# cvlab-kaist/SOLA

Hardware: AMD Instinct MI355X
Metric: track-selection forward+loss samples/sec at (T=32,N=64,d=256) (higher is better)
Workload: dtype f32 via split-f16 (hi+lo f16 operand pairs, 3 f16 MFMAs per product, f32 accumulate); 1 GPU; SOLA track selection forward+BCE+alignment loss+selection, T=32 N=64 d=256 L=16, mevis/default model (32.98M params, random init), 256 samples/step/GPU, conv weights re-standardised every step; batch_per_gpu=256, tracks=64, frames=32, text_len=16

## Files before the change

### include/sola_hip.h

```cpp
#ifndef SOLA_HIP_H
#define SOLA_HIP_H

#include <stddef.h>
#include <stdint.h>

#ifdef __cplusplus
extern "C" {
#endif

typedef enum SolaStatus {
    SOLA_OK = 0,
    SOLA_ERR_ARG = -1,
    SOLA_ERR_HIP = -2,
    SOLA_ERR_WEIGHT = -3,
    SOLA_ERR_WORKSPACE = -4,
    SOLA_ERR_STATE = -5
} SolaStatus;

typedef struct SolaConfig {
    int32_t object_token_dim;
    int32_t lang_token_dim;
    int32_t n_layers;
    int32_t max_temporal_length;
    int32_t n_negative;
// ... 14 lines not shown
int sola_weight_info(const SolaCtx* ctx, int index, const char** name, int64_t* numel);

int sola_set_weight(SolaCtx* ctx, const char* name, const void* dev_ptr, int64_t numel);

int sola_weights_changed(SolaCtx* ctx);
int sola_set_ws_policy(SolaCtx* ctx, int recompute_every_forward);

int sola_set_precision(SolaCtx* ctx, int precision);
int sola_set_split_guard(SolaCtx* ctx, int enable);

int sola_set_x16_arena(SolaCtx* ctx, void* dev_ptr, size_t bytes);
int sola_x16_arena_info(const SolaCtx* ctx, size_t* need_bytes, size_t* capacity_bytes, size_t* used_bytes);
int sola_split_fallback_count(const SolaCtx* ctx, int64_t* count, int32_t* last_guard);
int sola_cast_sp16(const float* dev_in, int ld_in, float* dev_out, int ld_out, int64_t rows, int K, float scale, void* stream);
int sola_cast_sp16_auto(const float* dev_in, int ld_in, float* dev_out, int ld_out, int64_t rows, int K, float* dev_scal, void* stream);
int sola_gemm_nt_split(const float* dev_a_sp, int lda, const float* dev_w_sp, const float* dev_bias, const float* dev_r,
                       int ldr, int r_is_split, float* dev_c, int ldc, int c_is_split, int M, int N, int K, float out_scale,
                       void* stream);
int sola_gemm_nt_split_scaled(const float* dev_a_sp, int lda, const float* dev_w_sp, const float* dev_bias, const float* dev_r,
                              int ldr, int r_is_split, float* dev_c, int ldc, int c_is_split, int M, int N, int K,
                              float out_scale, const float* dev_out_scale, void* stream);

int sola_cast_f16(const float* dev_in, int ld_in, void* dev_out, int ld_out, int64_t rows, int K, float scale, float* dev_scal, void* stream);
int sola_gemm_nt_f16(const void* dev_a_h, int lda, const void* dev_w_h, const float* dev_bias, const void* dev_r_h, int ldr,
                     void* dev_c, int ldc, int c_is_f16, int M, int N, int K, float out_scale, void* stream);
int sola_attention_f16(const void* dev_q, int ldq, const void* dev_k, int ldk, const void* dev_v, int ldv, void* dev_o, int ldo,
                       int G, int H, int head_dim, int Sq, int Sk, int inner, int64_t q_outer, int64_t q_inner, int64_t q_row_stride,
                       int64_t k_outer, int64_t k_inner, int64_t k_row_stride, float scale, void* stream);

int sola_gemm_nt_bf16(const void* dev_a, int lda, const void* dev_w, const float* dev_bias, const void* dev_r, int ldr, int r_is_bf16,
// ... 35 lines not shown

int sola_workspace_tap(const SolaCtx* ctx, const char* name, size_t* byte_offset, int64_t* rows, int64_t* cols);

int sola_loss(const float* dev_score_map, const float* dev_score_tokens,
              const float* dev_labels,
              const float* dev_pos_tokens,
              const float* dev_neg_tokens, int64_t neg_batch_stride,
              int B, int N, int D, int n_neg,
              float positive_weight, float temperature, float alignment_weight,
              float* dev_loss3, int32_t* dev_neg_argmax,
              void* dev_scratch, size_t scratch_bytes, void* stream);

int sola_select(const float* dev_score_map, int64_t n, float threshold, float* dev_prob, float* dev_pred, void* stream);

int sola_ws_standardize(const float* dev_w, int cout, int cin, int k, float* dev_out, void* stream);
int sola_gemm_nt(const float* dev_a, int lda, const float* dev_w, const float* dev_bias, const float* dev_r, int ldr,
                 float* dev_c, int ldc, int M, int N, int K, void* stream);
int sola_gemm_nn(const float* dev_a, int lda, const float* dev_w0, const float* dev_w1, const float* dev_w2, int w_rows, const float* dev_r,
                 int ldr, float* dev_c, int ldc, int M, int N, int K, void* stream);
int sola_conv1d_cl(const float* dev_x, const float* dev_wstd, const float* dev_bias, float* dev_y,
                   int R, int T_in, int cin, int cout, int k, int stride, int pad, void* stream);
int sola_group_norm(const float* dev_x, float* dev_y, float* dev_y2, const float* dev_pe,
                    const float* dev_gamma, const float* dev_beta,
                    int n_inst, int inner, int64_t outer_stride, int64_t inner_stride, int64_t tok_stride,
                    int ntok, int C, int groups, float eps, float leaky_slope, int apply_leaky, void* stream);
int sola_attention(const float* dev_q, int ldq, const float* dev_k, int ldk, const float* dev_v, int ldv,
                   float* dev_o, int ldo, int G, int H, int head_dim, int Sq, int Sk, int inner,
                   int64_t q_outer, int64_t q_inner, int64_t q_row_stride,
                   int64_t k_outer, int64_t k_inner, int64_t k_row_stride, float scale,
                   float* dev_lse , void* stream);
// ... 197 lines not shown
```

### sola_amd/_lib.py

```python
from __future__ import annotations

import contextlib
import ctypes as C
import os

_HERE = os.path.dirname(os.path.abspath(__file__))
LIB_PATH = os.environ.get("SOLA_HIP_LIB") or os.path.join(_HERE, "lib", "libsola_hip.so")


class SolaLibraryError(RuntimeError):
    pass


class SolaError(RuntimeError):
    """A libsola_hip call returned a negative status."""


class SolaConfig(C.Structure):
    _fields_ = [
        ("object_token_dim", C.c_int32),
        ("lang_token_dim", C.c_int32),
        ("n_layers", C.c_int32),
        ("max_temporal_length", C.c_int32),
        ("n_negative", C.c_int32),
# ... 20 lines not shown
    "sola_last_error": (C.c_char_p, []),
    "sola_version": (C.c_char_p, []),
    "sola_ctx_create": (_i, [C.POINTER(SolaConfig), _i, C.POINTER(_vp)]),
    "sola_ctx_destroy": (_i, [_vp]),
    "sola_num_weights": (_i, [_vp]),
    "sola_weight_info": (_i, [_vp, _i, C.POINTER(C.c_char_p), C.POINTER(_i64)]),
    "sola_set_weight": (_i, [_vp, C.c_char_p, _vp, _i64]),
    "sola_weights_changed": (_i, [_vp]),
    "sola_set_ws_policy": (_i, [_vp, _i]),
    "sola_set_precision": (_i, [_vp, _i]),
    "sola_set_split_guard": (_i, [_vp, _i]),
    "sola_split_fallback_count": (_i, [_vp, C.POINTER(_i64), C.POINTER(C.c_int32)]),
    "sola_cast_sp16": (_i, [_vp, _i, _vp, _i, _i64, _i, _f, _vp]),
    "sola_gemm_nt_split": (_i, [_vp, _i, _vp, _vp, _vp, _i, _i, _vp, _i, _i, _i, _i, _i, _f, _vp]),
    "sola_cast_sp16_auto": (_i, [_vp, _i, _vp, _i, _i64, _i, _vp, _vp]),
    "sola_gemm_nt_split_scaled": (_i, [_vp, _i, _vp, _vp, _vp, _i, _i, _vp, _i, _i, _i, _i, _i, _f, _vp, _vp]),
    "sola_cast_f16": (_i, [_vp, _i, _vp, _i, _i64, _i, _f, _vp, _vp]),
    "sola_gemm_nt_f16": (_i, [_vp, _i, _vp, _vp, _vp, _i, _vp, _i, _i, _i, _i, _i, _f, _vp]),
    "sola_gemm_nn": (_i, [_vp, _i, _vp, _vp, _vp, _i, _vp, _i, _vp, _i, _i, _i, _i, _vp]),
    "sola_gemm_nt_bf16": (_i, [_vp, _i, _vp, _vp, _vp, _i, _i, _vp, _i, _i, _i, _i, _i, _vp]),
    "sola_attention_bf16": (_i, [_vp, _i, _vp, _i, _vp, _i, _vp, _vp, _i, _i, _i, _i, _i, _i, _i, _i64, _i64, _i64, _i64, _i64, _i64, _f, _vp, _vp]),
    "sola_attention_backward_bf16": (_i, [_vp, _i, _vp, _i, _vp, _i, _vp, _i, _vp, _i, _i, _vp, _vp, _vp, _vp, _i, _i, _i, _vp, _vp, _i, _i, _i, _i, _i, _i,
                                          _i64, _i64, _i64, _i64, _i64, _i64, _f, _i64, _vp, _sz, _vp]),
    "sola_attention_f16": (_i, [_vp, _i, _vp, _i, _vp, _i, _vp, _i, _i, _i, _i, _i, _i, _i, _i64, _i64, _i64, _i64, _i64, _i64, _f, _vp]),
    "sola_workspace_bytes": (_sz, [_vp, _i, _i, _i, _i]),
    "sola_forward": (_i, [_vp, _vp, _vp, _i, _i, _i, _i, _vp, _vp, _vp, _sz, _vp]),
    "sola_ragged_workspace_bytes": (_sz, [_vp, C.POINTER(SolaRaggedBatch)]),
    "sola_forward_ragged": (_i, [_vp, _vp, _vp, C.POINTER(SolaRaggedBatch), _vp, _vp, _vp, _sz, _vp]),
    "sola_loss_ragged": (_i, [_vp, _vp, _vp, _vp, _vp, _i64, _i, _vp, _i, _i64, _i, _i, _f, _f, _f, _vp, _vp, _vp, _sz, _vp]),
    "sola_train_ragged_workspace_bytes": (_sz, [_vp, C.POINTER(SolaRaggedBatch)]),
    "sola_backward_ragged_workspace_bytes": (_sz, [_vp, C.POINTER(SolaRaggedBatch)]),
    "sola_forward_train_ragged": (_i, [_vp, _vp, _vp, C.POINTER(SolaRaggedBatch), _vp, _vp, _vp, _sz, _vp]),
    "sola_backward_ragged": (_i, [_vp, _vp, _vp, _vp, _vp, _sz, _vp]),
    "sola_loss_backward_ragged": (_i, [_vp, _vp, _vp, _vp, _vp, _i64, _i, _vp, _i, _i64, _i, _i, _f, _f, _f, _vp, _vp, _vp, _vp, _vp, _sz, _vp]),
    "sola_workspace_tap": (_i, [_vp, C.c_char_p, C.POINTER(_sz), C.POINTER(_i64), C.POINTER(_i64)]),
    "sola_loss": (_i, [_vp, _vp, _vp, _vp, _vp, _i64, _i, _i, _i, _i, _f, _f, _f, _vp, _vp, _vp, _sz, _vp]),
    "sola_select": (_i, [_vp, _i64, _f, _vp, _vp, _vp]),
    "sola_ws_standardize": (_i, [_vp, _i, _i, _i, _vp, _vp]),
    "sola_gemm_nt": (_i, [_vp, _i, _vp, _vp, _vp, _i, _vp, _i, _i, _i, _i, _vp]),
    "sola_conv1d_cl": (_i, [_vp, _vp, _vp, _vp, _i, _i, _i, _i, _i, _i, _i, _vp]),
    "sola_group_norm": (_i, [_vp, _vp, _vp, _vp, _vp, _vp, _i, _i, _i64, _i64, _i64, _i, _i, _i, _f, _f, _i, _vp]),
    "sola_attention": (_i, [_vp, _i, _vp, _i, _vp, _i, _vp, _i, _i, _i, _i, _i, _i, _i, _i64, _i64, _i64, _i64, _i64, _i64, _f, _vp, _vp]),
    "sola_attention_split": (_i, [_vp, _i, _vp, _i, _vp, _i, _vp, _i, _i, _i, _i, _i, _i, _i, _i, _i64, _i64, _i64, _i64, _i64, _i64, _f, _vp, _vp]),
    "sola_set_dropout": (_i, [_vp, _f, _f, C.c_uint64]),
    "sola_set_stage_dropout": (_i, [_f, C.c_uint64]),
    "sola_train_workspace_bytes": (_sz, [_vp, _i, _i, _i, _i]),
    "sola_backward_workspace_bytes": (_sz, [_vp, _i, _i, _i, _i]),
    "sola_set_grad": (_i, [_vp, C.c_char_p, _vp, _i64]),
    "sola_forward_train": (_i, [_vp, _vp, _vp, _i, _i, _i, _i, _vp, _vp, _vp, _sz, _vp]),
    "sola_backward": (_i, [_vp, _vp, _vp, _vp, _vp, _sz, _vp]),
    "sola_grad_bucket_count": (_i, [_vp]),
    "sola_grad_bucket_of": (_i, [_vp, C.c_char_p]),
    "sola_backward_wait_bucket": (_i, [_vp, _i, _vp]),
# ... 171 lines not shown
```

### sola_amd/csrc/api.hip

```cpp
#include <math.h>
#include <stdarg.h>
#include <string.h>

#include <algorithm>
#include <exception>
#include <mutex>

#include "ragged.h"
#include "tune.h"

static thread_local char g_err[1024] = "";
void sola_set_error(const char* fmt, ...) {
    va_list ap;
    va_start(ap, fmt);
    vsnprintf(g_err, sizeof(g_err), fmt, ap);
    va_end(ap);
}
extern "C" const char* sola_last_error(void) { return g_err; }
extern "C" const char* sola_version(void) { return "sola_hip 0.6 (gfx950; f32, range-guarded split-f16 and f16-operand MFMA forward and backward, ragged batches, mask IoU + masklet rows)"; }

namespace {
struct ProfRec {
    int cat;
    hipEvent_t e0, e1;
// ... 357 lines not shown
    if (rows) *rows = it->second.rows;
    if (cols) *cols = it->second.cols;
    return SOLA_OK;
}

extern "C" int sola_set_precision(SolaCtx* c, int precision) {
    SOLA_ARG(c && precision >= 0 && precision <= 3, "set_precision: 0 (f32), 1 (split-f16), 2 (f16 storage / f16 GEMM operands) or 3 (bf16 GEMM operands, training)");
    if (precision >= 1 && !c->lin16_buf) {
        const size_t D = c->cfg.lang_token_dim;
        size_t ws_total = 0;
        for (int i = 0; i < 6; ++i) ws_total += (size_t)c->conv[i].cout * c->conv[i].cin * c->conv[i].k;
        SOLA_HIP(hipSetDevice(c->device));
        SOLA_HIP(hipMalloc(&c->ws16_buf, ws_total * sizeof(float)));
        SOLA_HIP(hipMalloc(&c->lin16_buf, (size_t)c->cfg.n_layers * 12 * D * D * sizeof(float)));
        const size_t n_pairs = 2 + (size_t)c->cfg.n_layers * 12;
        SOLA_HIP(hipMalloc(&c->scal_buf, (2 * n_pairs + 2 + 4) * sizeof(float)));
        SOLA_HIP(hipMemset(c->scal_buf, 0, (2 * n_pairs + 2 + 4) * sizeof(float)));
        c->guard = reinterpret_cast<int*>(c->scal_buf + 2 * n_pairs);
        SOLA_HIP(hipHostMalloc(reinterpret_cast<void**>(&c->guard_host), 2 * sizeof(int), hipHostMallocDefault));
        c->guard_host[0] = c->guard_host[1] = 0;
    }
    c->precision = precision;
    c->ws_dirty = true;
    c->lin16_dirty = true;
    return SOLA_OK;
}

extern "C" int sola_cast_sp16(const float* in, int ld_in, float* out, int ld_out, int64_t rows, int K, float scale, void* stream_) {
    return launch_cast_sp16(in, ld_in, out, ld_out, rows, K, scale, as_stream(stream_));
}

extern "C" int sola_gemm_nt_split(const float* a_sp, int lda, const float* w_sp, const float* bias, const float* r, int ldr,
// ... 59 lines not shown
                                            int64_t q_rs, int64_t k_outer, int64_t k_inner, int64_t k_rs, float scale, int64_t q_rows, float* scratch,
                                            size_t scratch_floats, void* stream_) {
    SOLA_ARG(q && k && v && o && dout && lse && dq16 && dk16 && dv16 && dq_scratch && dvec, "attention_backward_bf16: null argument");
    AttnBwdDesc d{static_cast<const float*>(q), static_cast<const float*>(k), static_cast<const float*>(v), static_cast<const float*>(o), static_cast<const float*>(dout), lse, dq_scratch, nullptr, nullptr, dvec,
                  ldq, ldk, ldv, ldo, ld_dq, ld_dk, ld_dv, G, H, head_dim, Sq, Sk, inner, q_outer, q_inner, q_rs, k_outer, k_inner, k_rs, scale};
    d.drop = g_stage_drop;
    d.part = scratch; d.part_floats = scratch_floats; d.part_rows = q_rows;
    d.io_bf16 = 1; d.dq16 = dq16; d.dk16 = dk16; d.dv16 = dv16;
    d.dout_bf16 = dout_bf16 ? 1 : 0;
    d.o_bf16 = o_bf16 ? 1 : 0;
    return launch_attention_bwd(d, as_stream(stream_));
}

extern "C" int sola_cast_sp16_auto(const float* in, int ld_in, float* out, int ld_out, int64_t rows, int K, float* scal, void* stream_) {
    return launch_cast_sp16_auto(in, ld_in, out, ld_out, rows, K, scal, as_stream(stream_));
}

extern "C" int sola_gemm_nt_split_scaled(const float* a_sp, int lda, const float* w_sp, const float* bias, const float* r, int ldr,
                                         int r_sp16, float* cmat, int ldc, int c_sp16, int M, int N, int K, float out_scale,
                                         const float* out_scale_dev, void* stream_) {
    SOLA_ARG(a_sp && w_sp && cmat, "gemm_nt_split_scaled: null argument");
    GemmDesc gd{};
    gd.nprob = 1;
    gd.p[0] = GemmProblem{a_sp, w_sp, bias, r, cmat};
    gd.M = M; gd.N = N; gd.K = K; gd.lda = lda; gd.ldr = ldr; gd.ldc = ldc;
    gd.arith = 1; gd.out_scale = out_scale; gd.out_scale_dev = out_scale_dev; gd.r_sp16 = r_sp16; gd.c_sp16 = c_sp16;
    return launch_gemm(gd, as_stream(stream_));
}

int sola_split_guard_tripped(SolaCtx* c, hipStream_t s, bool* tripped) {
// ... 256 lines not shown

extern "C" int sola_grad_clip(float* const* dev_grads, const int64_t* numel, int n, const double* dev_total_sq,
                              float max_norm, void* stream_) {
    SOLA_ARG(dev_grads && numel && dev_total_sq, "grad_clip: null argument");
    return launch_mt_clip(dev_grads, reinterpret_cast<const long long*>(numel), n, dev_total_sq, max_norm, as_stream(stream_));
}

extern "C" int sola_select(const float* score, int64_t n, float thr, float* prob, float* pred, void* stream_) {
    SOLA_ARG(score && (prob || pred), "select: null argument");
    return launch_select(score, n, thr, prob, pred, as_stream(stream_));
}

extern "C" int sola_ws_standardize(const float* w, int cout, int cin, int k, float* out, void* stream_) {
    SOLA_ARG(w && out && cout > 0, "ws_standardize: bad argument");
    WsLayer l{w, out, cout, cin, k};
    return launch_ws_standardize(&l, 1, as_stream(stream_));
}

extern "C" int sola_ws_backward(const float* w, const float* dwstd, int cout, int cin, int k, float* dw, void* stream_) {
    SOLA_ARG(w && dwstd && dw && cout > 0, "ws_backward: bad argument");
    WsBwdLayer l{w, dwstd, dw, cout, cin, k};
    return launch_ws_backward(&l, 1, as_stream(stream_));
}

extern "C" int sola_gemm_nt(const float* a, int lda, const float* w, const float* bias, const float* r, int ldr,
                            float* cmat, int ldc, int M, int N, int K, void* stream_) {
    SOLA_ARG(a && w && cmat, "gemm_nt: null argument");
    GemmDesc gd{};
    gd.nprob = 1;
    gd.p[0] = GemmProblem{a, w, bias, r, cmat};
// ... 424 lines not shown
```

### sola_amd/csrc/cast.hip

```cpp
#include <algorithm>

#include "kernels.h"

namespace {

typedef _Float16 half8 __attribute__((ext_vector_type(8)));

__global__ __launch_bounds__(256) void cast_sp16_kernel(const float* __restrict__ in, float* __restrict__ out, long long rows,
                                                        int blocks_per_row, int ld_in, int ld_out, float scale, _Float16* __restrict__ side) {
    const long long i = (long long)blockIdx.x * blockDim.x + threadIdx.x;
    if (i >= rows * blocks_per_row) return;
    const long long r = i / blocks_per_row;
    const int b = (int)(i - r * blocks_per_row);
    const float4 v0 = *reinterpret_cast<const float4*>(in + r * ld_in + b * 8);
    const float4 v1 = *reinterpret_cast<const float4*>(in + r * ld_in + b * 8 + 4);
    const float v[8] = {v0.x * scale, v0.y * scale, v0.z * scale, v0.w * scale, v1.x * scale, v1.y * scale, v1.z * scale, v1.w * scale};
    half8 hi, lo;
#pragma unroll
    for (int j = 0; j < 8; ++j) {
        _Float16 h1, l1;
        split_f16(v[j], h1, l1);
        hi[j] = h1; lo[j] = l1;
    }
    half8* o = reinterpret_cast<half8*>(out + r * ld_out + b * 8);
// ... 120 lines not shown
    const long long r = i / blocks_per_row;
    const int b = (int)(i - r * blocks_per_row);
    const float4 v0 = *reinterpret_cast<const float4*>(in + r * ld_in + b * 8);
    const float4 v1 = *reinterpret_cast<const float4*>(in + r * ld_in + b * 8 + 4);
    const float v[8] = {v0.x * scale, v0.y * scale, v0.z * scale, v0.w * scale, v1.x * scale, v1.y * scale, v1.z * scale, v1.w * scale};
    half8 hi, lo;
#pragma unroll
    for (int j = 0; j < 8; ++j) {
        _Float16 h1, l1;
        split_f16(v[j], h1, l1);
        hi[j] = h1; lo[j] = l1;
    }
    half8* o = reinterpret_cast<half8*>(out + r * ld_out + b * 8);
    o[0] = hi;
    o[1] = lo;
}

constexpr int MULTI_MAX = 64;
struct MultiArgs {
    const float* in[MULTI_MAX];
    float* out[MULTI_MAX];
};
__global__ __launch_bounds__(256) void amax_multi_kernel(const MultiArgs a, unsigned* __restrict__ scal, long long n4) {
    const float* in = a.in[blockIdx.z];
    float m = 0.f;
    for (long long i = (long long)blockIdx.x * 256 + threadIdx.x; i < n4; i += (long long)gridDim.x * 256) {
        const float4 v = *reinterpret_cast<const float4*>(in + i * 4);
        m = fmaxf(m, fmaxf(fmaxf(fabsf(v.x), fabsf(v.y)), fmaxf(fabsf(v.z), fabsf(v.w))));
    }
    block_amax_commit(m, scal + 2 * blockIdx.z);
// ... 228 lines not shown
    SolaProfScope prof(SOLA_PROF_MISC, s, 0, 12.0 * rows * K);
    SOLA_HIP(hipMemsetAsync(scal, 0, 2 * sizeof(float), s));
    {
        long long ar = rows; int ak = K, ald = ld_in;
        amax_shape(ar, ak, ald);
        hipLaunchKernelGGL(amax_kernel, dim3((unsigned)((ak / 4 + 255) / 256), (unsigned)((ar + 63) / 64)), dim3(256), 0, s, in,
                           reinterpret_cast<unsigned*>(scal), ar, ak / 4, ald);
    }
    SOLA_LAUNCH_CHECK();
    const long long n = rows * (K / 8);
    hipLaunchKernelGGL(cast_sp16_auto_kernel, dim3((unsigned)((n + 255) / 256)), dim3(256), 0, s, in, out, rows, K / 8, ld_in, ld_out, scal);
    SOLA_LAUNCH_CHECK();
    return SOLA_OK;
}

int launch_cast_sp16(const float* in, int ld_in, float* out, int ld_out, long long rows, int K, float scale, hipStream_t s, void* side16) {
    SOLA_ARG(in && out && rows > 0 && K > 0 && K % 8 == 0 && ld_in % 4 == 0 && ld_out % 8 == 0, "cast_sp16: K=%d ld_in=%d ld_out=%d", K, ld_in, ld_out);
    const long long n = rows * (K / 8);
    SolaProfScope prof(SOLA_PROF_MISC, s, 0, (side16 ? 10.0 : 8.0) * rows * K);
    hipLaunchKernelGGL(cast_sp16_kernel, dim3((unsigned)((n + 255) / 256)), dim3(256), 0, s, in, out, rows, K / 8, ld_in, ld_out, scale,
                       static_cast<_Float16*>(side16));
    SOLA_LAUNCH_CHECK();
    return SOLA_OK;
}
```

### sola_amd/csrc/ctx.h

```cpp
#pragma once
#include <string>
#include <unordered_map>
#include <vector>

#include "kernels.h"

struct ConvGeom {
    int cin, cout, k, stride, pad;
};
struct Weight {
    std::string name;
    int64_t numel;
    const float* ptr;
    float* grad;
};
struct Buf {
    size_t off;
    int64_t rows, cols;
};
struct Plan {
    int B = 0, N = 0, T = 0, L = 0, W = 0, Tp = 0, M = 0;
    int Tl[6] = {0};
    bool train = false;
    bool rag = false;
// ... 70 lines not shown
    }
    float* scal_buf = nullptr;
    int* guard = nullptr;
    int* guard_host = nullptr;
    bool split_guard = true;
    long long split_fallbacks = 0;
    bool weight_range_bad = false;
    SolaRagStage* rag_stage = nullptr;
    std::vector<hipEvent_t> bucket_ev;
    hipStream_t side_stream = nullptr;
    hipEvent_t ev_fork = nullptr, ev_side[4] = {nullptr, nullptr, nullptr, nullptr};
    bool bucket_recorded = false;
    int n_buckets() const { return cfg.n_layers + 1; }
    float* scal_pair(int i) const { return scal_buf + 2 * i; }
    float* scal_extra(int i) const { return scal_buf + 2 * (2 + (size_t)cfg.n_layers * 12) + 2 + i; }
    const float* lin_inv_scale(int layer, int attn, int proj) const { return scal_buf + 2 * (2 + (layer * 3 + attn) * 4 + proj) + 1; }
    struct StepBinding {
        std::vector<int> widx;
        std::vector<int32_t> group;
        std::vector<long long> numel;
        int n_groups = 0;
        size_t sq_scratch = 0;
    } step;
    void* adam_tab = nullptr;
    int adam_n = 0, adam_cap = 0, adam_blocks = 0;
    bool adam_has_steps = false;
    int* adam_ticket = nullptr;
    double adam_bytes = 0.0;
    float p_drop_encoder = 0.f, p_drop_attention = 0.f;
    unsigned long long drop_seed = 0;
// ... 39 lines not shown
```

### sola_amd/csrc/forward_infer.hip

```cpp
#include <math.h>

#include <algorithm>

#include "ragged.h"

int sola_refresh_lin16(SolaCtx* c, hipStream_t s) {
    if (!c->lin16_dirty) return SOLA_OK;
    SOLA_ARG(c->lin16_buf && c->scal_buf, "split-f16 weights requested before sola_set_precision(ctx, 1)");
    static const char* pn[4] = {"q_proj", "k_proj", "v_proj", "out_proj"};
    const int D = c->cfg.lang_token_dim;
    std::vector<const float*> in;
    std::vector<float*> out;
    for (int l = 0; l < c->cfg.n_layers; ++l)
        for (int a = 0; a < 3; ++a)
            for (int j = 0; j < 4; ++j) {
                const std::string nm = "object_lang_align_layers." + std::to_string(l) + "." + kAttnLong[a] + "." + pn[j] + ".weight";
                const float* w = ctx_weight(c, nm);
                if (!w) {
                    sola_set_error("forward: weight '%s' has not been set", nm.c_str());
                    return SOLA_ERR_WEIGHT;
                }
                in.push_back(w);
                out.push_back(c->lin16_buf + ((size_t)(l * 3 + a) * 4 + j) * D * D);
            }
// ... 20 lines not shown
            return SOLA_ERR_WEIGHT;
        }
    SOLA_HIP(hipMemsetAsync(c->guard + 1, 0, sizeof(int), s));
    for (size_t i0 = 0; i0 < norms.size(); i0 += 32)
        SOLA_TRY(launch_norm_range_check(norms.data() + i0, (int)std::min<size_t>(32, norms.size() - i0), c->guard + 1, s));
    c->lin16_dirty = false;
    return SOLA_OK;
}

int sola_refresh_conv_weights(SolaCtx* c, int fmt, bool force, hipStream_t s) {
    if (!force && !c->ws_dirty && !c->ws_every_forward && (fmt == 0 || c->ws16_fmt == fmt)) return SOLA_OK;
    WsLayer layers[6];
    for (int i = 0; i < 6; ++i) {
        const std::string nm = "short_motion_encoder." + std::to_string(kConvIdx[i]) + ".weight";
        layers[i] = WsLayer{ctx_weight(c, nm), c->ws_buf + c->ws_off[i], c->conv[i].cout, c->conv[i].cin, c->conv[i].k};
    }
    SOLA_TRY(launch_ws_standardize(layers, 6, s));
    c->ws16_fmt = 0;
    for (int i = 0; i < 6 && fmt != 0; ++i) {
        const int kc = c->conv[i].k * c->conv[i].cin;
        const float* w = c->ws_buf + c->ws_off[i];
        if (fmt == 1) SOLA_TRY(launch_cast_sp16(w, kc, c->ws16_buf + c->ws_off[i], kc, c->conv[i].cout, kc, 1.f, s));
        else SOLA_TRY(launch_cast_f16(w, kc, reinterpret_cast<_Float16*>(c->ws16_buf) + c->ws_off[i], kc, c->conv[i].cout, kc, 1.f, nullptr, s, 13,
                                      nullptr, fmt == 3 ? 1 : 0));
    }
    c->ws_dirty = false;
    c->ws16_fmt = fmt;
    return SOLA_OK;
}

int sola_check_forward_args(const SolaCtx* c, const char* who, size_t need, const void* workspace, size_t ws_bytes) {
    for (const Weight& w : c->weights)
        if (!w.ptr) {
            sola_set_error("%s: weight '%s' has not been set", who, w.name.c_str());
            return SOLA_ERR_WEIGHT;
        }
// ... 63 lines not shown
    }
    std::string lin_name(int layer, int attn_i, int proj) const {
        return "object_lang_align_layers." + std::to_string(layer) + "." + kAttnLong[attn_i] + "." + kProj[proj];
    }
    GemmProblem lin_problem(const float* a, int layer, int attn_i, int proj, const float* r, float* out) const {
        const std::string nm = lin_name(layer, attn_i, proj);
        const size_t at = ((size_t)(layer * 3 + attn_i) * 4 + proj) * D * D;
        const float* w = sp ? c->lin16_buf + at
                       : h16 ? reinterpret_cast<const float*>(reinterpret_cast<const _Float16*>(c->lin16_buf) + at)
                             : W(nm + ".weight");
        return GemmProblem{a, w, W(nm + ".bias"), r, out, op16 ? c->lin_inv_scale(layer, attn_i, proj) : nullptr};
    }

    int cast_obj(const float* obj, float* obj_sp, long long rows) const {
        const int d_in = c->cfg.object_token_dim;
        if (sp) return launch_cast_sp16_auto(obj, d_in, obj_sp, d_in, rows, d_in, c->scal_pair(0), s);
        return launch_cast_f16(obj, d_in, obj_sp, d_in, rows, d_in, 256.f, c->scal_pair(0), s, 6, c->scal_extra(0));
    }
    int cast_lang(const float* lang, float* lang_sp, long long rows) const {
        if (sp) return launch_cast_sp16_auto(lang, D, lang_sp, D, rows, D, c->scal_pair(1), s);
        return launch_cast_f16(lang, D, lang_sp, D, rows, D, 1.f, c->scal_pair(1), s, 6);
    }
    const float* lang_inv_scale() const { return op16 ? c->scal_pair(1) + 1 : nullptr; }

    GemmDesc gemm(long long rows, int N, int K) const {
        GemmDesc gd{};
        gd.M = (int)rows; gd.N = N; gd.K = K; gd.ldc = N;
        if (op16) { gd.arith = sp ? 1 : 2; gd.out_scale = 1.f; }
        gd.splitk_ws = splitk_ws; gd.splitk_bytes = splitk_bytes;
        return gd;
    }
    GemmDesc conv_gemm(int i, const float* x, float* out, long long rows) const {
        const ConvGeom& g = c->conv[i];
        GemmDesc gd = gemm(rows, g.cout, g.k * g.cin);
        gd.nprob = 1;
// ... 376 lines not shown
```

### sola_amd/csrc/kernels.h

```cpp
#pragma once
#include "common.h"

struct GemmProblem {
    const float* A;
    const float* W;
    const float* bias;
    const float* R;
    float* C;
    const float* scale_dev;
};
struct GemmDesc {
    GemmProblem p[3];
    int nprob;
    int M, N, K;
    int lda, ldr, ldc;
    int conv;
    int T_in, T_out, stride, pad, Cin;
    const int2* rowmap;
    int arith;
    float out_scale;
    int ksplit;
    const float* out_scale_dev;
    int r_sp16;
    int c_sp16;
// ... 221 lines not shown

size_t mt_sqnorm_scratch_bytes(int n, const long long* numel);
int launch_mt_sqnorm(const float* const* ptrs, const long long* numel, const int* group, int n, int n_groups, double* out,
                     void* scratch, size_t scratch_bytes, hipStream_t s);
int launch_mt_clip(float* const* ptrs, const long long* numel, int n, const double* total_sq, float max_norm, hipStream_t s);
size_t mt_adam_entry_bytes();
void mt_adam_entry_fill(void* host_entry, float* p, float* g, float* m, float* v, float* step, long long numel, int first_block);
int mt_adam_blocks(long long numel);
int launch_mt_clip_adamw(const void* tab_dev, int n, int blocks, double bytes, const double* total_sq, float max_norm, double lr, double beta1, double beta2,
                         double eps, double weight_decay, float step, int write_back, int* ticket, hipStream_t s);

struct WsLayer {
    const float* w;
    float* out;
    int cout, cin, k;
};
int launch_ws_standardize(const WsLayer* layers, int n_layers, hipStream_t s);

struct GroupNormDesc {
    const float* x;
    float* y;
    float* y2;
    const float* pe;
    const float *gamma, *beta;
    int n_inst, inner;
    long long outer_stride, inner_stride, tok_stride;
    int ntok, C, groups;
    float eps, slope;
    int leaky;
    DropoutCfg drop;
// ... 6 lines not shown
    size_t slice_ws_bytes;
    void* y_cast = nullptr;
    void* y2_cast = nullptr;
    int cast_fmt = 0;
    void* stats_out = nullptr;
    int* stats_written = nullptr;
};
int launch_group_norm(const GroupNormDesc& d, hipStream_t s);
int launch_cast_sp16(const float* in, int ld_in, float* out, int ld_out, long long rows, int K, float scale, hipStream_t s, void* side16 = nullptr);
int launch_amax_accumulate(const float* in, int ld_in, long long rows, int K, float* scal, hipStream_t s);
int launch_amax_colsum(const float* in, int ld_in, long long rows, int K, float* scal, float* part, hipStream_t s);
int launch_cast_bf16_colsum(const float* in, int ld_in, void* out, int ld_out, long long rows, int K, float* scal, float* part, hipStream_t s);
int launch_colsum_slabs_bf16(const void* in, int ld_in, long long rows, int K, float* scal, float* part, hipStream_t s);
int launch_cast_sp16_scaled(const float* in, int ld_in, float* out, int ld_out, long long rows, int K, float* scal, hipStream_t s);
int launch_cast_sp16_auto(const float* in, int ld_in, float* out, int ld_out, long long rows, int K, float* scal, hipStream_t s);
int launch_cast_sp16_auto_multi(const float* const* in, float* const* out, int n, int rows, int K, float* scal, hipStream_t s);
int launch_cast_f16(const float* in, int ld_in, void* out, int ld_out, long long rows, int K, float scale, float* scal, hipStream_t s,
                    int target_exp = 13, float* scale_out = nullptr, int bf16 = 0);
int launch_cast_f16_auto_multi(const float* const* in, void* const* out, int n, int rows, int K, float* scal, hipStream_t s, int bf16 = 0);
int launch_cast_f16_scaled(const float* in, int ld_in, void* out, int ld_out, long long rows, int K, float* scal, hipStream_t s, int bf16 = 0);
int launch_cast_f16_t(const float* in, int ld_in, void* out, long long ld_out, int rows, int cols, float* scal, hipStream_t s, int bf16 = 0);
struct NormPair { const float *gamma, *beta; int C; };
int launch_norm_range_check(const NormPair* norms, int n, int* guard, hipStream_t s);
int launch_pos_encoding(const float* gauss, int D, int t_len, int max_len, float* pe, hipStream_t s);
int launch_lang_concat(const float* lang, const float* neg, float* out, float* lbar, int B, int L, int n_neg, int D,
                       hipStream_t s);
int launch_lang_concat_shared(const float* lang, const float* neg, float* out, float* lbar, int B, int L, int n_neg, int D, hipStream_t s);
int launch_lang_concat_ragged(const float* lang, const float* neg, float* out, float* lbar, int B, const int4* units, int n_neg,
                              int D, hipStream_t s);
int launch_gather_rows(const float* src, float* dst, const int4* list, int n, int row_floats, long long total_rows, hipStream_t s);
// ... 58 lines not shown
```

### sola_amd/csrc/norm.hip

```cpp
#include <algorithm>

#include <map>
#include <mutex>
#include <utility>

#include "kernels.h"

namespace {

constexpr int WS_MAX_LAYERS = 8;
constexpr int WS_MAX_PER_THREAD = 16;
struct WsArgs {
    WsLayer layer[WS_MAX_LAYERS];
    int first_block[WS_MAX_LAYERS + 1];
    int n_layers;
};

__global__ __launch_bounds__(256) void ws_standardize_kernel(const WsArgs a) {
    __shared__ float red[4];
    int li = 0;
    while (li + 1 < a.n_layers && (int)blockIdx.x >= a.first_block[li + 1]) ++li;
    const WsLayer L = a.layer[li];
    const int co = blockIdx.x - a.first_block[li];
    const int n = L.cin * L.k;
// ... 6 lines not shown
        v[i] = idx < n ? w[idx] : 0.f;
        s += v[i];
    }
    const float mean = block_sum_256(s, red) / (float)n;
    float q = 0.f;
#pragma unroll
    for (int i = 0; i < WS_MAX_PER_THREAD; ++i) {
        const int idx = threadIdx.x + 256 * i;
        const float c = idx < n ? v[i] - mean : 0.f;
        v[i] = c;
        q += c * c;
    }
    const float var = block_sum_256(q, red) / (float)(n - 1);
    const float denom = sqrtf(var) + 1e-5f;
    float* out = L.out + (long long)co * n;
#pragma unroll
    for (int i = 0; i < WS_MAX_PER_THREAD; ++i) {
        const int idx = threadIdx.x + 256 * i;
        if (idx < n) {
            const int ci = idx / L.k, kk = idx - ci * L.k;
            out[kk * L.cin + ci] = v[i] / denom;
        }
    }
}

struct GnArgs {
    const float* x;
    float* y;
    float* y2;
    const float* pe;
    const float *gamma, *beta;
    int inner;
    long long outer_stride, inner_stride, tok_stride;
    int ntok, C, cg, groups;
    float eps, slope;
    int leaky;
    DropoutCfg drop;
// ... 541 lines not shown
    const unsigned bx = (unsigned)std::max<long long>(1, std::min<long long>(64, (per + 1023) / 1024));
    hipLaunchKernelGGL(gather_rows_kernel, dim3(bx, n), dim3(256), 0, s, src, dst, list, row_floats / 4);
    SOLA_LAUNCH_CHECK();
    return SOLA_OK;
}

int launch_ws_standardize(const WsLayer* layers, int n_layers, hipStream_t s) {
    SOLA_ARG(n_layers >= 1 && n_layers <= WS_MAX_LAYERS, "ws: %d layers", n_layers);
    WsArgs a;
    a.n_layers = n_layers;
    int blocks = 0;
    double elems = 0;
    for (int i = 0; i < n_layers; ++i) {
        SOLA_ARG(layers[i].cin * layers[i].k <= 256 * WS_MAX_PER_THREAD && layers[i].cin * layers[i].k >= 2,
                 "ws: cin*k = %d unsupported (2..%d)", layers[i].cin * layers[i].k, 256 * WS_MAX_PER_THREAD);
        a.layer[i] = layers[i];
        a.first_block[i] = blocks;
        blocks += layers[i].cout;
        elems += (double)layers[i].cout * layers[i].cin * layers[i].k;
    }
    a.first_block[n_layers] = blocks;
    SolaProfScope prof(SOLA_PROF_WS, s, 6.0 * elems, 8.0 * elems);
    hipLaunchKernelGGL(ws_standardize_kernel, dim3(blocks), dim3(256), 0, s, a);
    SOLA_LAUNCH_CHECK();
    return SOLA_OK;
}

int g_gn_variant = 1;
int g_gn_wide = 1;
int g_gn_slices = 1;
// ... 114 lines not shown
```

Before: 18940 samples/s.

## Fuse split-f16 weight cast into WS standardize and carry input scale across steps

The conv weight standardization kernel now writes the hi/lo f16 split pairs directly from shared memory, so the separate per-layer cast launches are skipped. Object and language input casts switch to a carried-scale scheme: one pass computes the absmax and writes split values using the previous call's scale, and a settle kernel rewrites only when the new scale differs. This removes the separate absmax-then-cast round trip over the inputs. The cost is an extra shared buffer in the WS kernel, which may lower occupancy, and a rewrite pass whenever the scale changes between steps.

```diff
diff --git a/include/sola_hip.h b/include/sola_hip.h
--- a/include/sola_hip.h
+++ b/include/sola_hip.h
@@ -52,6 +52,8 @@
 int sola_split_fallback_count(const SolaCtx* ctx, int64_t* count, int32_t* last_guard);
 int sola_cast_sp16(const float* dev_in, int ld_in, float* dev_out, int ld_out, int64_t rows, int K, float scale, void* stream);
 int sola_cast_sp16_auto(const float* dev_in, int ld_in, float* dev_out, int ld_out, int64_t rows, int K, float* dev_scal, void* stream);
+int sola_cast_sp16_carried(const float* dev_in, int ld_in, float* dev_out, int ld_out, int64_t rows, int K, float* dev_scal,
+                           float* dev_carry, void* stream);
 int sola_gemm_nt_split(const float* dev_a_sp, int lda, const float* dev_w_sp, const float* dev_bias, const float* dev_r,
                        int ldr, int r_is_split, float* dev_c, int ldc, int c_is_split, int M, int N, int K, float out_scale,
                        void* stream);
@@ -117,6 +119,7 @@
 int sola_select(const float* dev_score_map, int64_t n, float threshold, float* dev_prob, float* dev_pred, void* stream);
 
 int sola_ws_standardize(const float* dev_w, int cout, int cin, int k, float* dev_out, void* stream);
+int sola_ws_standardize_split(const float* dev_w, int cout, int cin, int k, float* dev_out, float* dev_out_sp, void* stream);
 int sola_gemm_nt(const float* dev_a, int lda, const float* dev_w, const float* dev_bias, const float* dev_r, int ldr,
                  float* dev_c, int ldc, int M, int N, int K, void* stream);
 int sola_gemm_nn(const float* dev_a, int lda, const float* dev_w0, const float* dev_w1, const float* dev_w2, int w_rows, const float* dev_r,
diff --git a/sola_amd/_lib.py b/sola_amd/_lib.py
--- a/sola_amd/_lib.py
+++ b/sola_amd/_lib.py
@@ -58,6 +58,7 @@
     "sola_cast_sp16": (_i, [_vp, _i, _vp, _i, _i64, _i, _f, _vp]),
     "sola_gemm_nt_split": (_i, [_vp, _i, _vp, _vp, _vp, _i, _i, _vp, _i, _i, _i, _i, _i, _f, _vp]),
     "sola_cast_sp16_auto": (_i, [_vp, _i, _vp, _i, _i64, _i, _vp, _vp]),
+    "sola_cast_sp16_carried": (_i, [_vp, _i, _vp, _i, _i64, _i, _vp, _vp, _vp]),
     "sola_gemm_nt_split_scaled": (_i, [_vp, _i, _vp, _vp, _vp, _i, _i, _vp, _i, _i, _i, _i, _i, _f, _vp, _vp]),
     "sola_cast_f16": (_i, [_vp, _i, _vp, _i, _i64, _i, _f, _vp, _vp]),
     "sola_gemm_nt_f16": (_i, [_vp, _i, _vp, _vp, _vp, _i, _vp, _i, _i, _i, _i, _i, _f, _vp]),
@@ -81,6 +82,7 @@
     "sola_loss": (_i, [_vp, _vp, _vp, _vp, _vp, _i64, _i, _i, _i, _i, _f, _f, _f, _vp, _vp, _vp, _sz, _vp]),
     "sola_select": (_i, [_vp, _i64, _f, _vp, _vp, _vp]),
     "sola_ws_standardize": (_i, [_vp, _i, _i, _i, _vp, _vp]),
+    "sola_ws_standardize_split": (_i, [_vp, _i, _i, _i, _vp, _vp, _vp]),
     "sola_gemm_nt": (_i, [_vp, _i, _vp, _vp, _vp, _i, _vp, _i, _i, _i, _i, _vp]),
     "sola_conv1d_cl": (_i, [_vp, _vp, _vp, _vp, _i, _i, _i, _i, _i, _i, _i, _vp]),
     "sola_group_norm": (_i, [_vp, _vp, _vp, _vp, _vp, _vp, _i, _i, _i64, _i64, _i64, _i, _i, _i, _f, _f, _i, _vp]),
diff --git a/sola_amd/csrc/api.hip b/sola_amd/csrc/api.hip
--- a/sola_amd/csrc/api.hip
+++ b/sola_amd/csrc/api.hip
@@ -395,8 +395,8 @@
         SOLA_HIP(hipMalloc(&c->ws16_buf, ws_total * sizeof(float)));
         SOLA_HIP(hipMalloc(&c->lin16_buf, (size_t)c->cfg.n_layers * 12 * D * D * sizeof(float)));
         const size_t n_pairs = 2 + (size_t)c->cfg.n_layers * 12;
-        SOLA_HIP(hipMalloc(&c->scal_buf, (2 * n_pairs + 2 + 4) * sizeof(float)));
-        SOLA_HIP(hipMemset(c->scal_buf, 0, (2 * n_pairs + 2 + 4) * sizeof(float)));
+        SOLA_HIP(hipMalloc(&c->scal_buf, (2 * n_pairs + 2 + 8) * sizeof(float)));
+        SOLA_HIP(hipMemset(c->scal_buf, 0, (2 * n_pairs + 2 + 8) * sizeof(float)));
         c->guard = reinterpret_cast<int*>(c->scal_buf + 2 * n_pairs);
         SOLA_HIP(hipHostMalloc(reinterpret_cast<void**>(&c->guard_host), 2 * sizeof(int), hipHostMallocDefault));
         c->guard_host[0] = c->guard_host[1] = 0;
@@ -486,6 +486,10 @@
 
 extern "C" int sola_cast_sp16_auto(const float* in, int ld_in, float* out, int ld_out, int64_t rows, int K, float* scal, void* stream_) {
     return launch_cast_sp16_auto(in, ld_in, out, ld_out, rows, K, scal, as_stream(stream_));
+}
+
+extern "C" int sola_cast_sp16_carried(const float* in, int ld_in, float* out, int ld_out, int64_t rows, int K, float* scal, float* carry, void* stream_) {
+    return launch_cast_sp16_carried(in, ld_in, out, ld_out, rows, K, scal, carry, as_stream(stream_));
 }
 
 extern "C" int sola_gemm_nt_split_scaled(const float* a_sp, int lda, const float* w_sp, const float* bias, const float* r, int ldr,
@@ -772,6 +776,12 @@
 extern "C" int sola_ws_standardize(const float* w, int cout, int cin, int k, float* out, void* stream_) {
     SOLA_ARG(w && out && cout > 0, "ws_standardize: bad argument");
     WsLayer l{w, out, cout, cin, k};
+    return launch_ws_standardize(&l, 1, as_stream(stream_));
+}
+
+extern "C" int sola_ws_standardize_split(const float* w, int cout, int cin, int k, float* out, float* out_sp, void* stream_) {
+    SOLA_ARG(w && out && out_sp && cout > 0, "ws_standardize_split: bad argument");
+    WsLayer l{w, out, cout, cin, k, out_sp};
     return launch_ws_standardize(&l, 1, as_stream(stream_));
 }
 
diff --git a/sola_amd/csrc/cast.hip b/sola_amd/csrc/cast.hip
--- a/sola_amd/csrc/cast.hip
+++ b/sola_amd/csrc/cast.hip
@@ -1,5 +1,6 @@
 #include <algorithm>
 
+#include "cast_idx.h"
 #include "kernels.h"
 
 namespace {
@@ -158,6 +159,86 @@
     half8* o = reinterpret_cast<half8*>(out + r * ld_out + b * 8);
     o[0] = hi;
     o[1] = lo;
+}
+
+__global__ __launch_bounds__(kCarriedThreads) void cast_sp16_carried_kernel(const float* __restrict__ in, float* __restrict__ out, long long rows,
+                                                                            int blocks_per_row, int ld_in, int ld_out, float* __restrict__ scal,
+                                                                            float* __restrict__ carry) {
+    __shared__ float wmax[kCarriedThreads / 64];
+    const float scale = carry[0];
+    if (blockIdx.x == 0 && threadIdx.x == 0) carry[1] = scale;
+    const bool write = __float_as_uint(scale) != 0u;
+    const long long n = rows * blocks_per_row, step = sp16_walk_step(gridDim.x, kCarriedThreads);
+    float m = 0.f;
+    auto emit = [&](const Sp16Group& g, const float4& v0, const float4& v1) {
+        const float v[8] = {v0.x * scale, v0.y * scale, v0.z * scale, v0.w * scale, v1.x * scale, v1.y * scale, v1.z * scale, v1.w * scale};
+        half8 hi, lo;
+#pragma unroll
+        for (int j = 0; j < 8; ++j) {
+            _Float16 h1, l1;
+            split_f16(v[j], h1, l1);
+            hi[j] = h1; lo[j] = l1;
+        }
+        half8* o = reinterpret_cast<half8*>(out + g.out_off);
+        o[0] = hi;
+        o[1] = lo;
+    };
+    auto amax8 = [](const float4& v0, const float4& v1) {
+        return fmaxf(fmaxf(fmaxf(fabsf(v0.x), fabsf(v0.y)), fmaxf(fabsf(v0.z), fabsf(v0.w))),
+                     fmaxf(fmaxf(fabsf(v1.x), fabsf(v1.y)), fmaxf(fabsf(v1.z), fabsf(v1.w))));
+    };
+    for (long long i = sp16_walk_first(blockIdx.x, threadIdx.x, kCarriedThreads); i < n; i += 2 * step) {
+        const bool two = i + step < n;
+        const Sp16Group g0 = sp16_group(i, blocks_per_row, ld_in, ld_out);
+        const Sp16Group g1 = sp16_group(two ? i + step : i, blocks_per_row, ld_in, ld_out);
+        const float4 a0 = *reinterpret_cast<const float4*>(in + g0.in_off);
+        const float4 a1 = *reinterpret_cast<const float4*>(in + g0.in_off + 4);
+        const float4 b0 = *reinterpret_cast<const float4*>(in + g1.in_off);
+        const float4 b1 = *reinterpret_cast<const float4*>(in + g1.in_off + 4);
+        m = fmaxf(m, fmaxf(amax8(a0, a1), amax8(b0, b1)));
+        if (write) {
+            emit(g0, a0, a1);
+            if (two) emit(g1, b0, b1);
+        }
+    }
+#pragma unroll
+    for (int o = 32; o > 0; o >>= 1) m = fmaxf(m, __shfl_xor(m, o, 64));
+    if ((threadIdx.x & 63) == 0) wmax[threadIdx.x >> 6] = m;
+    __syncthreads();
+    if (threadIdx.x == 0) {
+#pragma unroll
+        for (int w = 1; w < kCarriedThreads / 64; ++w) m = fmaxf(m, wmax[w]);
+        if (m > 0.f && m <= 3.0e38f) atomicMax(reinterpret_cast<unsigned*>(scal), __float_as_uint(m));
+    }
+}
+
+__global__ __launch_bounds__(256) void cast_sp16_settle_kernel(const float* __restrict__ in, float* __restrict__ out, long long rows,
+                                                               int blocks_per_row, int ld_in, int ld_out, float* __restrict__ scal,
+                                                               float* __restrict__ carry) {
+    const float scale = auto_scale(reinterpret_cast<const unsigned*>(scal)[0]);
+    const float used = carry[1];
+    if (blockIdx.x == 0 && threadIdx.x == 0) {
+        scal[1] = 1.f / scale;
+        carry[0] = scale;
+    }
+    if (__float_as_uint(used) == __float_as_uint(scale)) return;
+    const long long n = rows * blocks_per_row, step = sp16_walk_step(gridDim.x, kSettleThreads);
+    for (long long i = sp16_walk_first(blockIdx.x, threadIdx.x, kSettleThreads); i < n; i += step) {
+        const Sp16Group g = sp16_group(i, blocks_per_row, ld_in, ld_out);
+        const float4 v0 = *reinterpret_cast<const float4*>(in + g.in_off);
+        const float4 v1 = *reinterpret_cast<const float4*>(in + g.in_off + 4);
+        const float v[8] = {v0.x * scale, v0.y * scale, v0.z * scale, v0.w * scale, v1.x * scale, v1.y * scale, v1.z * scale, v1.w * scale};
+        half8 hi, lo;
+#pragma unroll
+        for (int j = 0; j < 8; ++j) {
+            _Float16 h1, l1;
+            split_f16(v[j], h1, l1);
+            hi[j] = h1; lo[j] = l1;
+        }
+        half8* o = reinterpret_cast<half8*>(out + g.out_off);
+        o[0] = hi;
+        o[1] = lo;
+    }
 }
 
 constexpr int MULTI_MAX = 64;
@@ -416,6 +497,21 @@
     return SOLA_OK;
 }
 
+int launch_cast_sp16_carried(const float* in, int ld_in, float* out, int ld_out, long long rows, int K, float* scal, float* carry, hipStream_t s) {
+    SOLA_ARG(in && out && scal && carry && rows > 0 && K > 0 && K % 8 == 0 && ld_in % 4 == 0 && ld_out % 8 == 0,
+             "cast_sp16_carried: K=%d ld_in=%d ld_out=%d", K, ld_in, ld_out);
+    SolaProfScope prof(SOLA_PROF_MISC, s, 0, 8.0 * rows * K);
+    SOLA_HIP(hipMemsetAsync(scal, 0, 2 * sizeof(float), s));
+    const long long n = rows * (K / 8);
+    hipLaunchKernelGGL(cast_sp16_carried_kernel, dim3(sp16_walk_grid(n, kCarriedThreads, kCarriedBlocks)), dim3(kCarriedThreads), 0, s, in, out, rows, K / 8,
+                       ld_in, ld_out, scal, carry);
+    SOLA_LAUNCH_CHECK();
+    hipLaunchKernelGGL(cast_sp16_settle_kernel, dim3(sp16_walk_grid(n, kSettleThreads, kSettleBlocks)), dim3(kSettleThreads), 0, s, in, out, rows, K / 8,
+                       ld_in, ld_out, scal, carry);
+    SOLA_LAUNCH_CHECK();
+    return SOLA_OK;
+}
+
 int launch_cast_sp16(const float* in, int ld_in, float* out, int ld_out, long long rows, int K, float scale, hipStream_t s, void* side16) {
     SOLA_ARG(in && out && rows > 0 && K > 0 && K % 8 == 0 && ld_in % 4 == 0 && ld_out % 8 == 0, "cast_sp16: K=%d ld_in=%d ld_out=%d", K, ld_in, ld_out);
     const long long n = rows * (K / 8);
diff --git a/sola_amd/csrc/cast_idx.h b/sola_amd/csrc/cast_idx.h
--- /dev/null
+++ b/sola_amd/csrc/cast_idx.h
@@ -0,0 +1,31 @@
+#pragma once
+
+#if defined(__HIPCC__)
+#define SOLA_IDX __host__ __device__ inline
+#else
+#define SOLA_IDX inline
+#endif
+
+struct Sp16Group {
+    long long in_off, out_off;
+};
+SOLA_IDX Sp16Group sp16_group(long long i, int groups_per_row, int ld_in, int ld_out) {
+    const long long r = i / groups_per_row;
+    const long long b = i - r * groups_per_row;
+    return Sp16Group{r * ld_in + b * 8, r * ld_out + b * 8};
+}
+
+constexpr int kCarriedBlocks = 256, kCarriedThreads = 1024;
+constexpr int kSettleBlocks = 1024, kSettleThreads = 256;
+SOLA_IDX unsigned sp16_walk_grid(long long groups, int threads, int max_blocks) {
+    const long long blocks = (groups + threads - 1) / threads;
+    return (unsigned)(blocks < max_blocks ? blocks : max_blocks);
+}
+SOLA_IDX long long sp16_walk_first(unsigned block, unsigned thread, int threads) { return (long long)block * threads + thread; }
+SOLA_IDX long long sp16_walk_step(unsigned grid, int threads) { return (long long)grid * threads; }
+
+SOLA_IDX int ws_gemm_pos(int idx, int cin, int k) {
+    const int ci = idx / k, kk = idx - ci * k;
+    return kk * cin + ci;
+}
+SOLA_IDX int ws_groups(int n) { return n >> 3; }
diff --git a/sola_amd/csrc/ctx.h b/sola_amd/csrc/ctx.h
--- a/sola_amd/csrc/ctx.h
+++ b/sola_amd/csrc/ctx.h
@@ -108,6 +108,7 @@
     int n_buckets() const { return cfg.n_layers + 1; }
     float* scal_pair(int i) const { return scal_buf + 2 * i; }
     float* scal_extra(int i) const { return scal_buf + 2 * (2 + (size_t)cfg.n_layers * 12) + 2 + i; }
+    float* scal_carry(int t) const { return scal_extra(1 + 2 * t); }
     const float* lin_inv_scale(int layer, int attn, int proj) const { return scal_buf + 2 * (2 + (layer * 3 + attn) * 4 + proj) + 1; }
     struct StepBinding {
         std::vector<int> widx;
diff --git a/sola_amd/csrc/forward_infer.hip b/sola_amd/csrc/forward_infer.hip
--- a/sola_amd/csrc/forward_infer.hip
+++ b/sola_amd/csrc/forward_infer.hip
@@ -58,12 +58,14 @@
     for (int i = 0; i < 6; ++i) {
         const std::string nm = "short_motion_encoder." + std::to_string(kConvIdx[i]) + ".weight";
         layers[i] = WsLayer{ctx_weight(c, nm), c->ws_buf + c->ws_off[i], c->conv[i].cout, c->conv[i].cin, c->conv[i].k};
+        if (fmt == 1 && (c->conv[i].k * c->conv[i].cin) % 8 == 0 && c->ws_off[i] % 4 == 0) layers[i].out_sp = c->ws16_buf + c->ws_off[i];
     }
     SOLA_TRY(launch_ws_standardize(layers, 6, s));
     c->ws16_fmt = 0;
     for (int i = 0; i < 6 && fmt != 0; ++i) {
         const int kc = c->conv[i].k * c->conv[i].cin;
         const float* w = c->ws_buf + c->ws_off[i];
+        if (layers[i].out_sp) continue;
         if (fmt == 1) SOLA_TRY(launch_cast_sp16(w, kc, c->ws16_buf + c->ws_off[i], kc, c->conv[i].cout, kc, 1.f, s));
         else SOLA_TRY(launch_cast_f16(w, kc, reinterpret_cast<_Float16*>(c->ws16_buf) + c->ws_off[i], kc, c->conv[i].cout, kc, 1.f, nullptr, s, 13,
                                       nullptr, fmt == 3 ? 1 : 0));
@@ -157,11 +159,11 @@
 
     int cast_obj(const float* obj, float* obj_sp, long long rows) const {
         const int d_in = c->cfg.object_token_dim;
-        if (sp) return launch_cast_sp16_auto(obj, d_in, obj_sp, d_in, rows, d_in, c->scal_pair(0), s);
+        if (sp) return launch_cast_sp16_carried(obj, d_in, obj_sp, d_in, rows, d_in, c->scal_pair(0), c->scal_carry(0), s);
         return launch_cast_f16(obj, d_in, obj_sp, d_in, rows, d_in, 256.f, c->scal_pair(0), s, 6, c->scal_extra(0));
     }
     int cast_lang(const float* lang, float* lang_sp, long long rows) const {
-        if (sp) return launch_cast_sp16_auto(lang, D, lang_sp, D, rows, D, c->scal_pair(1), s);
+        if (sp) return launch_cast_sp16_carried(lang, D, lang_sp, D, rows, D, c->scal_pair(1), c->scal_carry(1), s);
         return launch_cast_f16(lang, D, lang_sp, D, rows, D, 1.f, c->scal_pair(1), s, 6);
     }
     const float* lang_inv_scale() const { return op16 ? c->scal_pair(1) + 1 : nullptr; }
diff --git a/sola_amd/csrc/kernels.h b/sola_amd/csrc/kernels.h
--- a/sola_amd/csrc/kernels.h
+++ b/sola_amd/csrc/kernels.h
@@ -259,6 +259,7 @@
     const float* w;
     float* out;
     int cout, cin, k;
+    float* out_sp = nullptr;
 };
 int launch_ws_standardize(const WsLayer* layers, int n_layers, hipStream_t s);
 
@@ -295,6 +296,7 @@
 int launch_colsum_slabs_bf16(const void* in, int ld_in, long long rows, int K, float* scal, float* part, hipStream_t s);
 int launch_cast_sp16_scaled(const float* in, int ld_in, float* out, int ld_out, long long rows, int K, float* scal, hipStream_t s);
 int launch_cast_sp16_auto(const float* in, int ld_in, float* out, int ld_out, long long rows, int K, float* scal, hipStream_t s);
+int launch_cast_sp16_carried(const float* in, int ld_in, float* out, int ld_out, long long rows, int K, float* scal, float* carry, hipStream_t s);
 int launch_cast_sp16_auto_multi(const float* const* in, float* const* out, int n, int rows, int K, float* scal, hipStream_t s);
 int launch_cast_f16(const float* in, int ld_in, void* out, int ld_out, long long rows, int K, float scale, float* scal, hipStream_t s,
                     int target_exp = 13, float* scale_out = nullptr, int bf16 = 0);
diff --git a/sola_amd/csrc/norm.hip b/sola_amd/csrc/norm.hip
--- a/sola_amd/csrc/norm.hip
+++ b/sola_amd/csrc/norm.hip
@@ -4,6 +4,7 @@
 #include <mutex>
 #include <utility>
 
+#include "cast_idx.h"
 #include "kernels.h"
 
 namespace {
@@ -44,13 +45,32 @@
     const float var = block_sum_256(q, red) / (float)(n - 1);
     const float denom = sqrtf(var) + 1e-5f;
     float* out = L.out + (long long)co * n;
+    __shared__ float row[256 * WS_MAX_PER_THREAD];
 #pragma unroll
     for (int i = 0; i < WS_MAX_PER_THREAD; ++i) {
         const int idx = threadIdx.x + 256 * i;
         if (idx < n) {
-            const int ci = idx / L.k, kk = idx - ci * L.k;
-            out[kk * L.cin + ci] = v[i] / denom;
-        }
+            const int p = ws_gemm_pos(idx, L.cin, L.k);
+            const float y = v[i] / denom;
+            out[p] = y;
+            if (L.out_sp) row[p] = y;
+        }
+    }
+    if (!L.out_sp) return;
+    __syncthreads();
+    typedef _Float16 ws_half8 __attribute__((ext_vector_type(8)));
+    float* sp = L.out_sp + (long long)co * n;
+    for (int g = threadIdx.x; g < ws_groups(n); g += 256) {
+        ws_half8 hi, lo;
+#pragma unroll
+        for (int j = 0; j < 8; ++j) {
+            _Float16 h1, l1;
+            split_f16(row[g * 8 + j], h1, l1);
+            hi[j] = h1; lo[j] = l1;
+        }
+        ws_half8* o = reinterpret_cast<ws_half8*>(sp + g * 8);
+        o[0] = hi;
+        o[1] = lo;
     }
 }
 
@@ -622,6 +642,8 @@
     for (int i = 0; i < n_layers; ++i) {
         SOLA_ARG(layers[i].cin * layers[i].k <= 256 * WS_MAX_PER_THREAD && layers[i].cin * layers[i].k >= 2,
                  "ws: cin*k = %d unsupported (2..%d)", layers[i].cin * layers[i].k, 256 * WS_MAX_PER_THREAD);
+        SOLA_ARG(!layers[i].out_sp || ((layers[i].cin * layers[i].k) % 8 == 0 && (reinterpret_cast<uintptr_t>(layers[i].out_sp) & 15) == 0),
+                 "ws: split pairs need cin*k = %d to be a multiple of 8 and a 16-byte aligned output", layers[i].cin * layers[i].k);
         a.layer[i] = layers[i];
         a.first_block[i] = blocks;
         blocks += layers[i].cout;
```

New measurement: 19060 samples/s (median of 6 runs). Within noise of the previous version (+0.7%).
